# MichelangeloConserva/Colosseum

Hardware: AMD Instinct MI355X
Metric: env steps/sec (whole node) + value-iteration sweeps/sec, DeepSea size=30 x65536 (higher is better)
Workload: dtype i32 state/visit indices, f64 rewards+CDF

## Files before the change

### colosseum_amd/_lib.py

```python
import ctypes as C
import os

import numpy as np

HERE = os.path.dirname(os.path.abspath(__file__))
LIB_PATH = os.path.join(HERE, "libcmdp.so")

OK, ERR_INVALID, ERR_HIP, ERR_NEEDS_RESET, ERR_UNSUPPORTED, ERR_MAX_ITER, ERR_NO_DEVICE, ERR_MAX_VALUE, ERR_OVERFLOW = (
    0, -1, -2, -3, -4, -5, -6, -7, -8)
RNG_MT_COMPAT, RNG_PHILOX = 0, 1
POLICY_RANDOM, POLICY_HOST_ACTIONS, POLICY_GREEDY_Q = 0, 1, 2
POLICY_RANDOM_REFERENCE = 3
SCHEME_AUTO, SCHEME_JACOBI, SCHEME_GAUSS_SEIDEL = 0, 1, 2
LAYOUT_CSR, LAYOUT_DENSE = 0, 1
FLAG_REWARD_MEANS = 1
FLAG_BETA_GAMMAS = 4
FLAG_REWARD_CACHE = 2
OPT_ROLLOUT_KERNEL = 1
OPT_DP_KERNEL = 2
OPT_LDS_GROUPS_PER_CU = 3
OPT_DIAMETER_WORKSPACE_MB = 4
OPT_CHAIN_EXACT_ORDER = 5
OPT_MIXING_PATH = 6
OPT_DIAMETER_RELABEL_MIN_STATES = 7
# ... 5 lines not shown
STAT_UCRL2_WAIT_MS = 16
STAT_PSRL_ROUNDS, STAT_PSRL_SOLVES, STAT_PSRL_SAMPLE_KERNEL_MS, STAT_PSRL_VI_KERNEL_MS, STAT_PSRL_REFERENCE_MS = 17, 18, 19, 20, 21
STAT_DIAMETER_KERNEL = 22
STAT_UCRL2_POLICY_KERNEL_MS = 23
STAT_PSRL_POLICY_KERNEL_MS = 24
STAT_UCRL2_POLICY_SOLVED, STAT_UCRL2_POLICY_REUSED = 25, 26
STAT_ACTIONS_KERNEL_MS = 27
STAT_PSRL_UNCONVERGED, STAT_PSRL_SWEEPS = 28, 29
PSRLC_OPT_SIZE_THRESHOLD, PSRLC_OPT_MAX_SWEEPS, PSRLC_OPT_POLICY_SOLVER = 1, 2, 3
PSRL_SAMPLER_REFERENCE, PSRL_SAMPLER_PHILOX = 0, 1
PSRL_KEY_HI = 0x5053524C
BOUND_CHERNOFF, BOUND_BERNSTEIN = 0, 1
ACTOR_GREEDY, ACTOR_EPSILON_GREEDY, ACTOR_BOLTZMANN = 0, 1, 2
UCRL2_OPT_MAX_SWEEPS = 1
UCRL2_OPT_POLICY_SIZE_THRESHOLD = 2
UCRL2_OPT_POLICY_REUSE = 3
NOISE_NONE, NOISE_GAUSSIAN, NOISE_GAUSSIAN_CORRELATED, NOISE_STUDENT_T, NOISE_STUDENT_T_CORRELATED = 0, 1, 2, 3, 4
CALIB_LDS_READ, CALIB_LDS_CHAIN, CALIB_LDS_CHAIN_SHARED = 0, 1, 2
DP_AUTO, DP_WORKGROUP, DP_REGISTER = 0, 1, 2
DP_REGISTER_DISTINCT = 5
DP_REGISTER_WAVEFRONT = 7
ROLLOUT_AUTO, ROLLOUT_GLOBAL, ROLLOUT_LDS, ROLLOUT_LDS_STOCHASTIC = 0, 1, 2, 3
ROLLOUT_LDS_TEMPLATE = 4
ROLLOUT_LDS_TEMPLATE_STREAM = 5
ROLLOUT_EPISODE_PARALLEL = 6
K1S_PLAN_FIELDS = ("ok", "G", "nw", "gw", "team", "U", "n_pat", "n_codes", "reward_mode", "rc_packed", "n_shapes", "shape_bytes",
                   "ch", "form")
K1S_REWARD_SOURCES = ("packed", "state_table", "row")
K1S_FORMS = {0: "generic", **{t * 4 + i: f"team{t}_{src}" for t in (16, 8, 1) for i, src in enumerate(K1S_REWARD_SOURCES)}}
DET_PLAN_FIELDS = {
    "k1lp": ("ok", "pipe", "packed", "code_shift", "succ_bits", "n_codes", "ch", "G", "per_cu", "capacity", "slot_bytes", "lds_bytes",
             "form"),
    "k1t": ("ok", "automatic", "ch", "G", "capacity", "slot_bytes", "tmpl_bytes", "lds_bytes"),
    "k1u": ("ok", "automatic", "pack10", "ch", "G", "capacity", "lds_bytes", "hist_lds_bytes", "form"),
}
K1LP_FORMS = {0: "k1l_unpacked", 1: "k1l_packed", 2: "k1p"}
K1U_FORMS = {0: "pack10", 1: "wide"}
K1E_PAIR_PLAN_FIELDS = ("ok", "H", "SP2", "n_even", "lds_bytes", "last_form")
K1E_FORMS = {0: None, 1: "single", 2: "pair"}
DET_PLAN_KNOBS = ("pipe", "k1l_G", "k1t_G", "k1u_G", "k1t_ch")

EXPORTS = [
    "cmdp_version", "cmdp_build_id", "cmdp_last_error", "cmdp_device_count", "cmdp_set_device", "cmdp_create", "cmdp_destroy",
    "cmdp_stream", "cmdp_reset", "cmdp_step", "cmdp_rollout", "cmdp_rollout_async", "cmdp_synchronize", "cmdp_stat", "cmdp_calibrate", "cmdp_set_option", "cmdp_lds_plan",
    "cmdp_visits", "cmdp_reset_visits", "cmdp_set_visits", "cmdp_state", "cmdp_last_start", "cmdp_vi_discounted", "cmdp_pe_discounted",
    "cmdp_vi_episodic", "cmdp_pe_episodic", "cmdp_diameter", "cmdp_diameter_episodic", "cmdp_value_norm", "cmdp_gth", "cmdp_qlearning_create", "cmdp_qlearning_destroy", "cmdp_qlearning_run",
    "cmdp_qlearning_tables", "cmdp_qlearning_evaluate", "cmdp_greedy_policy_episodic", "cmdp_qlearning_continuous_create",
    "cmdp_qlearning_policy", "cmdp_qlearning_average_reward", "cmdp_qlearning_run_logged", "cmdp_tracker_replay", "cmdp_average_reward", "cmdp_diameter_range", "cmdp_diameter_sparse_f64", "cmdp_mixing_time", "cmdp_set_observation_table", "cmdp_observe", "cmdp_observe_noise",
    "cmdp_set_reward_streams", "cmdp_legacy_beta", "cmdp_extended_vi",
    "cmdp_ucrl2_create", "cmdp_ucrl2_destroy", "cmdp_ucrl2_run", "cmdp_ucrl2_layout", "cmdp_ucrl2_model", "cmdp_ucrl2_last_solve",
    "cmdp_ucrl2_set_option", "cmdp_ucrl2_policy", "cmdp_ucrl2_average_reward", "cmdp_model_vi_scheme", "cmdp_vi_discounted_model",
    "cmdp_psrl_create", "cmdp_psrl_destroy", "cmdp_psrl_run", "cmdp_psrl_layout", "cmdp_psrl_model", "cmdp_psrl_last_sample",
    "cmdp_psrl_reference_sample", "cmdp_vi_episodic_dense", "cmdp_psrl_episode_end_update", "cmdp_k1e_round_interior",
    "cmdp_k1e_code_counts", "cmdp_k1e_scan_words", "cmdp_k1s_plan", "cmdp_k1s_plan_desc", "cmdp_det_plan", "cmdp_det_plan_desc", "cmdp_chain_plan_desc", "cmdp_chain_choice",
    "cmdp_k1e_pair_plan", "cmdp_k1e_pair_plan_desc",
    "cmdp_psrl_map_rows", "cmdp_vi_episodic_map", "cmdp_psrl_policy", "cmdp_psrl_evaluate",
    "cmdp_ucrl2_run_logged", "cmdp_psrl_run_logged",
    "cmdp_set_action_streams", "cmdp_action_stream_state", "cmdp_set_action_stream_state", "cmdp_mt_randint", "cmdp_mt_action_bits",
    "cmdp_psrlc_create", "cmdp_psrlc_destroy", "cmdp_psrlc_run", "cmdp_psrlc_episode_end_update", "cmdp_psrlc_layout",
    "cmdp_psrlc_model", "cmdp_psrlc_last_sample", "cmdp_psrlc_set_option", "cmdp_psrlc_policy", "cmdp_psrlc_average_reward",
    "cmdp_vi_discounted_dense", "cmdp_vi_discounted_map",
]


class CmdpDesc(C.Structure):
    _fields_ = [
        ("n_instances", C.c_int32), ("n_actions", C.c_int32), ("horizon", C.c_int32), ("rng_mode", C.c_int32),
        ("layout", C.c_int32), ("flags", C.c_int32),
        ("reward_min", C.c_double), ("reward_max", C.c_double),
        ("state_off", C.c_void_p),
        ("sp_ptr", C.c_void_p), ("sp_next", C.c_void_p), ("sp_cum", C.c_void_p), ("sp_reward", C.c_void_p),
        ("sp_rkind", C.c_void_p), ("sp_rp0", C.c_void_p), ("sp_rp1", C.c_void_p), ("sp_seed", C.c_void_p), ("start_off", C.c_void_p), ("start_state", C.c_void_p),
        ("start_cum", C.c_void_p), ("start_seed", C.c_void_p), ("philox_key", C.c_void_p),
        ("csr_ptr", C.c_void_p), ("csr_col", C.c_void_p), ("csr_val", C.c_void_p), ("R", C.c_void_p),
    ]


class CmdpLoopDesc(C.Structure):
    _fields_ = [
        ("n_steps", C.c_int64), ("log_every", C.c_int64),
        ("n_check", C.c_int32), ("horizon", C.c_int32), ("kmax", C.c_int32), ("reserved", C.c_int32),
        ("max_time", C.c_double),
        ("base_val", C.c_void_p), ("base_kind", C.c_void_p), ("opt0", C.c_void_p), ("worst0", C.c_void_p),
        ("start_pos", C.c_void_p), ("start_prob", C.c_void_p),
    ]


LOG_COLUMNS = [
    "cumulative_expected_reward", "cumulative_regret", "cumulative_reward", "normalized_cumulative_expected_reward",
    "normalized_cumulative_regret", "normalized_cumulative_reward", "optimal_cumulative_expected_reward",
    "optimal_normalized_cumulative_expected_reward", "random_cumulative_expected_reward", "random_cumulative_regret",
    "random_normalized_cumulative_expected_reward", "random_normalized_cumulative_regret", "steps_per_second",
    "worst_cumulative_expected_reward", "worst_cumulative_regret", "worst_normalized_cumulative_expected_reward",
    "worst_normalized_cumulative_regret",
]


class CmdpError(RuntimeError):
    def __init__(self, code, message):
        super().__init__(f"libcmdp error {code}: {message}")
        self.code = code


class DynamicProgrammingMaxIterationExceeded(Exception):
    """Same name as the reference's exception (colosseum/dynamic_programming/utils.py:8-9)."""


# ... 88 lines not shown
        L.cmdp_diameter_sparse_f64.argtypes = [vp, C.c_double, i64, vp, vp]
        L.cmdp_mixing_time.argtypes = [vp, vp, vp, C.c_double, i64, vp, vp]
        L.cmdp_set_observation_table.argtypes = [vp, vp, i32, i32]
        L.cmdp_observe.argtypes = [vp, C.c_double, vp]
        L.cmdp_observe_noise.argtypes = [vp, i32, C.c_double, C.c_double, vp, vp]
        L.cmdp_greedy_policy_episodic.argtypes = [vp, i32, i32, vp, vp]
        L.cmdp_qlearning_tables.argtypes = [vp, vp, vp]
        L.cmdp_set_reward_streams.argtypes = [vp, vp, vp, vp, vp]
        L.cmdp_legacy_beta.argtypes = [vp, vp, vp, vp, f64, f64, i64, vp]
        L.cmdp_set_action_streams.argtypes = [vp, vp]
        L.cmdp_action_stream_state.argtypes = [vp, vp, vp]
        L.cmdp_set_action_stream_state.argtypes = [vp, vp, vp]
        L.cmdp_mt_randint.argtypes = [vp, vp, i32, i64, vp]
        L.cmdp_mt_action_bits.argtypes = [vp, vp, i64, i64, vp]
        L.cmdp_ucrl2_create.argtypes = [C.POINTER(vp), vp, vp, i64, f64, f64, i32, i32, i32]
        L.cmdp_ucrl2_destroy.argtypes = [vp]
        L.cmdp_ucrl2_run.argtypes = [vp, i64, i32, vp, vp, vp, vp, vp, vp]
        L.cmdp_ucrl2_layout.argtypes = [vp, vp, vp, vp]
        L.cmdp_ucrl2_model.argtypes = [vp, vp, vp, vp, vp, vp, vp, vp, vp, vp]
        L.cmdp_ucrl2_last_solve.argtypes = [vp, vp, vp, vp, vp, vp, vp, vp, vp, vp]
        L.cmdp_ucrl2_set_option.argtypes = [vp, i32, i64]
        L.cmdp_ucrl2_policy.argtypes = [vp, vp, vp, vp, vp, vp]
        L.cmdp_ucrl2_average_reward.argtypes = [vp, vp, vp, vp]
        L.cmdp_model_vi_scheme.argtypes = [i32, i32, i64, i64, f64]
        L.cmdp_vi_discounted_model.argtypes = [i32, vp, vp, vp, vp, vp, vp, vp, f32, f64, i32, i64, f64, i64, vp, vp, vp, vp, vp]
        L.cmdp_psrl_create.argtypes = [C.POINTER(vp), vp, vp, i64, vp, vp, i32, i32]
        L.cmdp_psrl_destroy.argtypes = [vp]
        L.cmdp_psrl_run.argtypes = [vp, i64, i32, vp, vp, vp, vp, vp, vp]
        L.cmdp_psrl_episode_end_update.argtypes = [vp]
        L.cmdp_psrl_layout.argtypes = [vp, vp, vp, vp]
        L.cmdp_psrl_model.argtypes = [vp, vp, vp, vp, vp]
        L.cmdp_psrl_last_sample.argtypes = [vp, vp, vp, vp]
        L.cmdp_psrl_reference_sample.argtypes = [vp, vp, vp, vp, vp, vp, vp, vp, i32, i32, vp, vp, vp, vp, f32, vp, vp, vp]
        L.cmdp_vi_episodic_dense.argtypes = [i32, vp, vp, i32, vp, vp, vp, vp]
        L.cmdp_psrl_map_rows.argtypes = [i32, i32, vp, vp, vp, f32, vp, vp, vp]
        L.cmdp_vi_episodic_map.argtypes = [i32, vp, vp, i32, vp, vp, vp, vp, vp, vp, vp, vp, vp]
        L.cmdp_psrl_policy.argtypes = [vp, vp, vp, vp]
        L.cmdp_psrl_evaluate.argtypes = [vp, vp, vp]
        L.cmdp_psrlc_create.argtypes = [C.POINTER(vp), vp, vp, i64, vp, vp, i32, i32]
        L.cmdp_psrlc_destroy.argtypes = [vp]
        L.cmdp_psrlc_run.argtypes = [vp, i64, i32, vp, vp, vp, vp, vp, vp]
        L.cmdp_psrlc_episode_end_update.argtypes = [vp]
        L.cmdp_psrlc_layout.argtypes = [vp, vp, vp, vp]
        L.cmdp_psrlc_model.argtypes = [vp, vp, vp, vp, vp, vp, vp]
        L.cmdp_psrlc_last_sample.argtypes = [vp, vp, vp, vp, vp, vp, vp]
        L.cmdp_psrlc_set_option.argtypes = [vp, i32, i64]
        L.cmdp_psrlc_policy.argtypes = [vp, vp, vp, vp, vp, vp]
        L.cmdp_psrlc_average_reward.argtypes = [vp, vp, vp, vp]
        L.cmdp_vi_discounted_dense.argtypes = [i32, vp, vp, vp, vp, f32, f64, i32, i64, f64, i64, vp, vp, vp, vp, vp]
        L.cmdp_vi_discounted_map.argtypes = [i32, vp, vp, vp, vp, vp, vp, vp, f32, f64, i32, i64, f64, i64, vp, vp, vp, vp, vp, vp, vp]
        L.cmdp_k1e_round_interior.argtypes = [i32, i32, i64, i32]
        L.cmdp_k1e_code_counts.argtypes = [C.c_uint32, C.c_uint32, i32]
        L.cmdp_k1e_scan_words.argtypes = [vp, i64, i32, i32, i64, i32, i32, vp, f64, vp, vp]
        L.cmdp_k1s_plan.argtypes = [vp, vp]
        L.cmdp_k1s_plan_desc.argtypes = [C.POINTER(CmdpDesc), i32, i32, vp]
        L.cmdp_det_plan.argtypes = [vp, vp]
        L.cmdp_det_plan_desc.argtypes = [C.POINTER(CmdpDesc), i32, vp, vp]
        L.cmdp_k1e_pair_plan.argtypes = [vp, vp]
        L.cmdp_k1e_pair_plan_desc.argtypes = [C.POINTER(CmdpDesc), i32, i32, vp, vp, vp, vp, vp]
        L.cmdp_chain_plan_desc.argtypes = [C.POINTER(CmdpDesc), vp, vp, vp, vp, i64, vp, vp, vp, vp, vp]
        L.cmdp_chain_choice.argtypes = [i32, i32, i32, i32, i32, vp]
        L.cmdp_k1e_code_counts.restype = C.c_uint32
        _lib = L
    return _lib


def check(rc):
    if rc == OK:
        return
    msg = load().cmdp_last_error().decode()
    if rc == ERR_MAX_ITER:
        raise DynamicProgrammingMaxIterationExceeded(msg)
    if rc == ERR_NEEDS_RESET:
        raise AssertionError(msg)
    raise CmdpError(rc, msg)


def ptr(a):
    return None if a is None else a.ctypes.data_as(C.c_void_p)


def carr(a, dtype):
    return None if a is None else np.ascontiguousarray(a, dtype)


_hip = None


def pinned_empty(n, dtype):
    import weakref

    global _hip
    load()
    if _hip is None:
        _hip = C.CDLL("libamdhip64.so")
        _hip.hipHostMalloc.argtypes = [C.POINTER(C.c_void_p), C.c_size_t, C.c_uint]
        _hip.hipHostFree.argtypes = [C.c_void_p]
    dt = np.dtype(dtype)
    nbytes = max(1, int(n)) * dt.itemsize
    p = C.c_void_p()
    rc = _hip.hipHostMalloc(C.byref(p), nbytes, 0)
    if rc != 0 or not p.value:
        raise MemoryError(f"hipHostMalloc({nbytes}) failed with {rc}")
    buf = (C.c_char * nbytes).from_address(p.value)
    arr = np.frombuffer(buf, dtype=dt, count=int(n))
    weakref.finalize(buf, _hip.hipHostFree, C.c_void_p(p.value))
# ... 2 lines not shown
```

### colosseum_amd/csrc/cmdp.hip

```cpp
#include "../../include/cmdp.h"

#include <hip/hip_runtime.h>
#include <rocblas/rocblas.h>
#include <cstdlib>

#include <algorithm>
#include <chrono>
#include <cstdarg>
#include <limits>
#include <cstdio>
#include <cmath>
#include <cstring>
#include <map>
#include <memory>
#include <mutex>
#include <string>
#include <unordered_map>
#include <vector>

extern char** environ;

#include <new>
#include "cmdp_kernels.h"
#include "cmdp_tracker.h"
// ... 706 lines not shown
  }
  HIP_TRY(h->d_csr_ptr.upload(d->csr_ptr, R + 1, st));
  HIP_TRY(h->d_csr_col.upload(d->csr_col, N, st));
  HIP_TRY(h->d_csr_val.upload(d->csr_val, N, st));
  HIP_TRY(h->d_R.upload(d->R, R, st));
  return CMDP_OK;
}

static int build_dense(cmdp_t* h, const cmdp_desc* d) {
  const int64_t R = h->n_rows;
  for (int64_t k = 0; k < h->n_csr; ++k)
    if (!(d->csr_val[k] >= 3.7252902984619141e-09f) || d->csr_val[k] > 1.0f)
      return fail(CMDP_ERR_INVALID, "dense layout needs probabilities in [2^-28, 1] (entry %lld)", (long long)k);
  const int nv = (h->max_S + 255) / 256;
  const int allowed[] = {1, 2, 3, 4, 6, 8, 12, 16};
  int pick = 0;
  for (int v : allowed) if (v >= nv) { pick = v; break; }
  if (!pick) return fail(CMDP_ERR_UNSUPPORTED, "dense layout supports at most 4096 states per instance");
  h->dense_spad = pick * 256;
  const size_t n = (size_t)R * h->dense_spad;
  size_t free_b = 0, total_b = 0;
  HIP_TRY(hipMemGetInfo(&free_b, &total_b));
  if (n * sizeof(float) > free_b)
    return fail(CMDP_ERR_INVALID, "dense layout needs %zu MiB, %zu MiB free", n * sizeof(float) >> 20, free_b >> 20);
  HIP_TRY(h->d_dense.alloc(n));
  HIP_TRY(h->d_dense.zero(h->stream));
  hipLaunchKernelGGL(k_dense_fill, dim3(grid_for(R, 256)), dim3(256), 0, h->stream, h->d_dense.p, h->dense_spad,
                     h->d_csr_ptr.p, h->d_csr_col.p, h->d_csr_val.p, R);
  HIP_TRY(hipGetLastError());
  return CMDP_OK;
}

extern "C" {

int cmdp_version(void) { return CMDP_ABI_VERSION; }
#ifndef CMDP_BUILD_ID
#define CMDP_BUILD_ID "unstamped"
#endif
static const char k_build_id[] = "CMDP_BUILD_ID=" CMDP_BUILD_ID;
const char* cmdp_build_id(void) { return k_build_id + 14; }

const char* cmdp_last_error(void) { return g_err.c_str(); }

int cmdp_k1e_round_interior(int e_lo, int horizon, int64_t n_steps, int n_instances) {
  return k1e_round_interior(e_lo, horizon, n_steps, n_instances) ? 1 : 0;
}

uint32_t cmdp_k1e_code_counts(uint32_t lo, uint32_t hi, int few) {
  return few ? k1e_code_counts_few(lo, hi) : k1e_code_counts(lo, hi);
}

int cmdp_k1e_scan_words(const uint64_t* words, int64_t n_words, int H, int h0, int64_t n_steps, int nch, int n_codes,
                        const double rv[4], double s0, double* sum, int32_t stats[4]) {
  if (!words || !rv || !sum || !stats) return fail(CMDP_ERR_INVALID, "cmdp_k1e_scan_words: null argument");
  if (H < 1 || h0 < 0 || h0 >= H || n_steps < 1 || n_steps >= ((int64_t)1 << 31) || nch != (H + 31) / 32 || n_codes < 1 || n_codes > 4)
    return fail(CMDP_ERR_INVALID, "cmdp_k1e_scan_words: H %d, h0 %d, n_steps %lld, nch %d, n_codes %d", H, h0, (long long)n_steps, nch, n_codes);
  if ((((int64_t)h0 + n_steps + H - 1) / H) * nch != n_words || n_words >= ((int64_t)1 << 31))
    return fail(CMDP_ERR_INVALID, "cmdp_k1e_scan_words: %lld words do not hold %lld steps from in-episode time %d", (long long)n_words,
                (long long)n_steps, h0);
  double r[4];
  for (int c = 0; c < 4; ++c) r[c] = c < n_codes ? rv[c] : 0.0;
  K1rLane L;
  k1r_init(L, r, n_codes, H, nch, h0, n_steps, s0);
  K1rHostLoader ld{words, L.W};
  K1rStats st;
  k1r_scan(L, ld, st);
  *sum = k1r_sum(L);
  for (int i = 0; i < 4; ++i) stats[i] = st.n[i];
  return CMDP_OK;
}

int cmdp_device_count(void) {
  int n = 0;
  if (hipGetDeviceCount(&n) != hipSuccess) return 0;
  return n;
}

int cmdp_set_device(int device) {
  HIP_TRY(hipSetDevice(device));
  if (const char* e = std::getenv("CMDP_SYNC_MODE")) {
    const unsigned f = !std::strcmp(e, "block") ? hipDeviceScheduleBlockingSync
                     : !std::strcmp(e, "yield") ? hipDeviceScheduleYield
                     : !std::strcmp(e, "spin") ? hipDeviceScheduleSpin : hipDeviceScheduleAuto;
    HIP_TRY(hipSetDeviceFlags(f));
  }
  return CMDP_OK;
}

void* cmdp_stream(cmdp_t* h) { return h ? (void*)h->stream : nullptr; }

int cmdp_destroy(cmdp_t* h) {
  if (h && h->ev_dp0) {
    (void)hipEventDestroy(h->ev_dp0);
    (void)hipEventDestroy(h->ev_dp1);
  }
  if (!h) return CMDP_OK;
  (void)hipSetDevice(h->device);
  if (h->stream) {
    (void)hipStreamSynchronize(h->stream);
    (void)hipStreamDestroy(h->stream);
  }
  for (int i = 0; i < 2; ++i) {
    if (h->aux.walk[i]) (void)hipEventDestroy(h->aux.walk[i]);
    if (h->aux.scan[i]) (void)hipEventDestroy(h->aux.scan[i]);
  }
  if (h->aux.stream) {
    (void)hipStreamSynchronize(h->aux.stream);
    (void)hipStreamDestroy(h->aux.stream);
  }
  for (int i = 0; i < 5; ++i)
    if (h->ev_time[i]) (void)hipEventDestroy(h->ev_time[i]);
  for (int i = 0; i < 2; ++i)
    if (h->ev_row[i]) (void)hipEventDestroy(h->ev_row[i]);
  for (int i = 0; i < 2; ++i)
    if (h->ev_as[i]) (void)hipEventDestroy(h->ev_as[i]);
  for (cmdp_t** back : h->uc_backrefs) *back = nullptr;
  for (double* c : h->rc_chunks) (void)hipFree(c);
  if (h->rc_stage_h) (void)hipHostFree(h->rc_stage_h);
  if (h->rc_dst_h) (void)hipHostFree(h->rc_dst_h);
  if (h->rc_ent_h) (void)hipHostFree(h->rc_ent_h);
  if (h->rc_list_h) (void)hipHostFree(h->rc_list_h);
// ... 4845 lines not shown
```

### colosseum_amd/csrc/cmdp_k1e.h

```cpp
#pragma once

#define K1E_THREADS 1024
#define K1E_NW (K1E_THREADS / 64)
#define K1E_NI 32
#define K1E_EPL 4
#define K1E_EPP (K1E_NW * 2 * K1E_EPL)
#define K1E_SEG 61440
#define K1E_SMASK 0xff80u

struct K1ePlan {
  int32_t S, H;
  int32_t ash;
  int32_t ring_blocks;
  int32_t n_codes;
  int32_t nch;
  int32_t n_pass;
  int32_t gdw;
  int32_t debug;
  int32_t fast;
  const uint32_t* etab;
  const double* rvals;
  uint2* codes;
  int32_t* seg_h0;
  int2* dep;
// ... 408 lines not shown
    }
  }
  __syncthreads();
  const int64_t so0 = t.state_off[g0];
  bool ovf = false;
  auto sat_add = [&](int32_t old, uint32_t add) -> int32_t {
    const int64_t v = (int64_t)old + (int64_t)add;
    if (v > 0x7fffffffLL) { ovf = true; return 0x7fffffff; }
    return (int32_t)v;
  };
  for (int i = wave; i < nb; i += K1E_NW) {
    const int bi = g0 + i;
    const int32_t s_start = t.start_state[t.start_off[bi]];
    const uint32_t n_res = (uint32_t)p.dep_res[bi];
    const int64_t gs0 = so0 + (int64_t)i * S;
    for (int s = lane; s < S; s += 64) {
      const uint32_t c0 = arr0[i * S + s], c1 = arr1[i * S + s];
      const uint32_t add_s = c0 + c1 + (s == s_start ? n_res : 0u);
      if (add_s) t.visits_s[gs0 + s] = sat_add(t.visits_s[gs0 + s], add_s);
      if (c0 | c1) {
        int2* sa = reinterpret_cast<int2*>(t.visits_sa + (gs0 + s) * 2);
        int2 v = *sa;
        v.x = sat_add(v.x, c0);
        v.y = sat_add(v.y, c1);
        *sa = v;
      }
    }
    __builtin_amdgcn_wave_barrier();
    if (lane == 0) p.dep_res[bi] = 0;
  }
  if (ovf) atomicOr(overflow, 1);
}

typedef uint32_t k1r_u32x8 __attribute__((ext_vector_type(8)));
__host__ __device__ __forceinline__ uint32_t k1r_sel8(const k1r_u32x8 a, int i) {
  const bool i0 = (i & 1) != 0, i1 = (i & 2) != 0, i2 = (i & 4) != 0;
  const uint32_t b0 = i0 ? a[1] : a[0], b1 = i0 ? a[3] : a[2], b2 = i0 ? a[5] : a[4], b3 = i0 ? a[7] : a[6];
  const uint32_t c0 = i1 ? b1 : b0, c1 = i1 ? b3 : b2;
  return i2 ? c1 : c0;
}

typedef uint32_t k1r_u32x4 __attribute__((ext_vector_type(4)));
__host__ __device__ __forceinline__ uint32_t k1r_sel8h(const k1r_u32x4 a, int i) {
  const bool i1 = (i & 2) != 0, i2 = (i & 4) != 0;
  const uint32_t b0 = i1 ? a[1] : a[0], b1 = i1 ? a[3] : a[2];
  return ((i2 ? b1 : b0) >> ((i & 1) << 4)) & 0xffffu;
}

#define K1R_THREADS 64
#define K1R_T 8
#define K1R_D 3
#if defined(__HIP_DEVICE_COMPILE__)
#define K1R_ALL(x) (__all(x) != 0)
#else
#define K1R_ALL(x) (x)
#endif

struct K1rNoStats {
  __host__ __device__ __forceinline__ void plain() {}
  __host__ __device__ __forceinline__ void slow() {}
  __host__ __device__ __forceinline__ void word() {}
  __host__ __device__ __forceinline__ void rebase() {}
};
struct K1rStats {
  int32_t n[4] = {0, 0, 0, 0};
  void plain() { ++n[0]; }
  void slow() { ++n[1]; }
  void word() { ++n[2]; }
  void rebase() { ++n[3]; }
};

struct K1rLane {
  double rv[4];
  unsigned long long mv[4];
  int eb[4];
  bool bulk_allowed;
  int n_codes, H, nch;
  int W;
  bool kvalid;
  int kb;
  unsigned long long m;
  uint32_t qlo[4], qhi[4];
  uint32_t tie;
  int ch;
  int e_len;
  int ep_left;
  int tot_left;
};

__host__ __device__ __forceinline__ void k1r_rebase(K1rLane& L) {
  const unsigned long long M52 = (1ull << 52) - 1ull, B52 = 1ull << 52;
  L.kvalid = false;
  const unsigned long long sb = L.m;
  const double S = __builtin_bit_cast(double, sb);
  if (!L.bulk_allowed || !(S >= 2.2250738585072014e-308) || !(S < 1.0e300)) return;
  L.kb = (int)(sb >> 52);
  L.m = (sb & M52) | B52;
  L.tie = 0u;
#pragma unroll
  for (int c = 0; c < 4; ++c) {
    if (c < L.n_codes) {
      unsigned long long qq = 0ull;
      if (L.rv[c] != 0.0) {
        const int d = L.kb - L.eb[c];
        if (L.eb[c] == 0 || d < 0) L.tie |= 1u << c;
        else if (d == 0) qq = L.mv[c];
        else if (d < 55) {
          const unsigned long long half = 1ull << (d - 1), rem = L.mv[c] & ((1ull << d) - 1ull);
          qq = (L.mv[c] >> d) + (rem > half ? 1ull : 0ull);
          if (rem == half) L.tie |= 1u << c;
        }
      }
      L.qlo[c] = (uint32_t)qq;
      L.qhi[c] = (uint32_t)(qq >> 32);
    }
  }
  L.kvalid = true;
}

__host__ __device__ __forceinline__ void k1r_init(K1rLane& L, const double (&rv)[4], int n_codes, int H, int nch, int h0,
                                                  int64_t n_steps, double S0) {
  const unsigned long long M52 = (1ull << 52) - 1ull, B52 = 1ull << 52;
// ... 13 lines not shown
  L.m = __builtin_bit_cast(unsigned long long, S0);
  L.kvalid = false; L.kb = 0; L.tie = 0u;
  L.ch = 0;
  L.e_len = (int)((int64_t)(H - h0) < n_steps ? (int64_t)(H - h0) : n_steps);
  L.ep_left = L.e_len;
  L.tot_left = (int)n_steps;
  k1r_rebase(L);
}

__host__ __device__ __forceinline__ bool k1r_advance(const K1rLane& L, uint32_t n1, uint32_t n2, uint32_t n3, uint32_t steps,
                                                     unsigned long long& m2) {
  const uint32_t n0 = steps - n1 - n2 - n3;
  const uint32_t present = (n0 ? 1u : 0u) | (n1 ? 2u : 0u) | (n2 ? 4u : 0u) | (n3 ? 8u : 0u);
  unsigned long long lo64 = (unsigned long long)n0 * L.qlo[0];
  lo64 += (unsigned long long)n1 * L.qlo[1];
  lo64 += (unsigned long long)n2 * L.qlo[2];
  lo64 += (unsigned long long)n3 * L.qlo[3];
  const uint32_t hi32 = n0 * L.qhi[0] + n1 * L.qhi[1] + n2 * L.qhi[2] + n3 * L.qhi[3];
  m2 = L.m + lo64 + ((unsigned long long)hi32 << 32);
  return L.kvalid && (present & L.tie) == 0u && m2 < (1ull << 53);
}
__host__ __device__ __forceinline__ bool k1r_advance(const K1rLane& L, uint32_t nw, uint32_t steps, unsigned long long& m2) {
  return k1r_advance(L, nw & 0x7ffu, (nw >> 11) & 0x7ffu, nw >> 22, steps, m2);
}
__host__ __device__ __forceinline__ unsigned long long k1r_compose(const K1rLane& L) {
  return ((unsigned long long)L.kb << 52) | (L.m & ((1ull << 52) - 1ull));
}
__host__ __device__ __forceinline__ double k1r_sum(const K1rLane& L) {
  return __builtin_bit_cast(double, L.kvalid ? k1r_compose(L) : L.m);
}

__host__ __device__ __forceinline__ void k1r_tile_counts_few(const k1r_u32x8& clo, const k1r_u32x8& chi, uint32_t& n1, uint32_t& n2) {
  uint32_t n12 = 0u, c2 = 0u;
#pragma unroll
  for (int k = 0; k < K1R_T; ++k) {
    n12 += (uint32_t)__builtin_popcount(clo[k]);
    n12 += (uint32_t)__builtin_popcount(chi[k]);
    c2 += (uint32_t)__builtin_popcount((clo[k] & 0xaaaaaaaau) | ((chi[k] >> 1) & 0x55555555u));
  }
  n1 = n12 - c2; n2 = c2;
}
__host__ __device__ __forceinline__ void k1r_tile_counts(const k1r_u32x8& clo, const k1r_u32x8& chi, uint32_t& n1, uint32_t& n2,
                                                         uint32_t& n3) {
  uint32_t all = 0u, odd = 0u, c3 = 0u;
#pragma unroll
  for (int k = 0; k < K1R_T; ++k) {
    all += (uint32_t)__builtin_popcount(clo[k]);
    all += (uint32_t)__builtin_popcount(chi[k]);
    odd += (uint32_t)__builtin_popcount((clo[k] & 0xaaaaaaaau) | ((chi[k] >> 1) & 0x55555555u));
    const uint32_t l3 = clo[k] & (clo[k] >> 1), h3 = chi[k] & (chi[k] >> 1);
    c3 += (uint32_t)__builtin_popcount((l3 & 0x55555555u) | ((h3 << 1) & 0xaaaaaaaau));
  }
  n3 = c3; n2 = odd - c3; n1 = all - odd - c3;
}

template <class ST>
__host__ __device__ __forceinline__ void k1r_slow(K1rLane& L, const k1r_u32x8& clo, const k1r_u32x8& chi, const k1r_u32x8& P,
                                                  const k1r_u32x4& SP, ST& st) {
  const uint32_t Pt = P[K1R_T - 1], St = SP[K1R_T / 2 - 1] >> 16;
  const double rv0 = L.rv[0], rv1 = L.rv[1], rv2 = L.rv[2], rv3 = L.rv[3];
  unsigned long long m2;
  uint32_t base_n = 0u, base_s = 0u;
  int from = 0;
  for (;;) {
    int lo = from, hi = K1R_T - 1;
#pragma unroll
    for (int it = 0; it < 3; ++it) {
      const int mid = (lo + hi) >> 1;
      const bool ok = k1r_advance(L, k1r_sel8(P, mid) - base_n, k1r_sel8h(SP, mid) - base_s, m2);
      if (lo < hi) { if (ok) lo = mid + 1; else hi = mid; }
    }
    const int k = lo;
    const uint32_t Sk1 = k > 0 ? k1r_sel8h(SP, k - 1) : 0u;
    if (k > from && k1r_advance(L, k1r_sel8(P, k - 1) - base_n, Sk1 - base_s, m2)) L.m = m2;
    const uint32_t Sk = k1r_sel8h(SP, k);
    const uint32_t Lw = Sk - Sk1;
    if (Lw) {
      st.word();
      const uint32_t cx = k1r_sel8(clo, k), cy = k1r_sel8(chi, k);
      double S = __builtin_bit_cast(double, L.kvalid ? k1r_compose(L) : L.m);
#pragma unroll
      for (int half = 0; half < 2; ++half) {
        const uint32_t cw = half ? cy : cx;
        const int Lh = (int)Lw - 16 * half;
        if (Lh > 0) {
          const uint32_t vm = Lh >= 16 ? 0x55555555u : ((1u << (2 * Lh)) - 1u) & 0x55555555u;
          const uint32_t b0 = cw & vm, b1 = (cw >> 1) & vm;
          uint32_t nz = 0u;
          if (rv0 != 0.0) nz |= vm & ~(b0 | b1);
          if (rv1 != 0.0) nz |= b0 & ~b1;
          if (rv2 != 0.0) nz |= b1 & ~b0;
          if (rv3 != 0.0) nz |= b0 & b1;
          while (nz) {
            const uint32_t pos = (uint32_t)__builtin_ctz(nz);
            nz &= nz - 1u;
            const uint32_t cd = cw >> pos;
            const bool c0 = (cd & 1u) != 0u, c1 = (cd & 2u) != 0u;
            const double lo2 = c0 ? rv1 : rv0, hi2 = c0 ? rv3 : rv2;
            S += c1 ? hi2 : lo2;
          }
        }
      }
      L.m = __builtin_bit_cast(unsigned long long, S);
      k1r_rebase(L);
      st.rebase();
    }
    base_n = k1r_sel8(P, k);
    base_s = Sk;
    from = k + 1;
    if (from >= K1R_T) break;
    if (k1r_advance(L, Pt - base_n, St - base_s, m2)) { L.m = m2; break; }
  }
}

template <class ST>
__host__ __device__ __forceinline__ void k1r_tile(K1rLane& L, const k1r_u32x8& clo, const k1r_u32x8& chi, const int w0, ST& st) {
  const int H = L.H;
  const bool few = L.n_codes <= 3;
  unsigned long long m2;
  k1r_u32x8 P;
  k1r_u32x4 SP;
  const bool plain = L.nch == 1 && K1R_ALL(w0 >= 1 && w0 + K1R_T <= L.W - 1);
  if (plain) {
    uint32_t n1, n2, n3;
    bool whole;
    if (few) {
      k1r_tile_counts_few(clo, chi, n1, n2);
      whole = k1r_advance(L, n1, n2, 0u, (uint32_t)(K1R_T * H), m2);
    } else {
      k1r_tile_counts(clo, chi, n1, n2, n3);
      whole = k1r_advance(L, n1, n2, n3, (uint32_t)(K1R_T * H), m2);
    }
    L.tot_left -= K1R_T * H;
    L.e_len = H < L.tot_left ? H : L.tot_left;
    L.ep_left = L.e_len;
    if (whole) { L.m = m2; st.plain(); return; }
  }
  uint32_t rn[K1R_T];
  if (few) {
#pragma unroll
    for (int k = 0; k < K1R_T; ++k) rn[k] = k1e_code_counts_few(clo[k], chi[k]);
  } else {
#pragma unroll
    for (int k = 0; k < K1R_T; ++k) rn[k] = k1e_code_counts(clo[k], chi[k]);
  }
  if (plain) {
    uint32_t acc = 0u;
#pragma unroll
    for (int k = 0; k < K1R_T; ++k) { acc += rn[k]; P[k] = acc; }
#pragma unroll
    for (int k = 0; k < K1R_T; k += 2) SP[k >> 1] = (uint32_t)((k + 1) * H) | ((uint32_t)((k + 2) * H) << 16);
  } else {
    uint32_t acc = 0u, sacc = 0u;
#pragma unroll
    for (int k = 0; k < K1R_T; ++k) {
      const int Lk = (w0 + k < L.W) ? (L.ep_left < 0 ? 0 : (L.ep_left < 32 ? L.ep_left : 32)) : 0;
      acc += Lk > 0 ? rn[k] : 0u;
      sacc += (uint32_t)Lk;
      P[k] = acc;
      if (k & 1) SP[k >> 1] |= sacc << 16; else SP[k >> 1] = sacc;
      L.ep_left -= 32;
      if (++L.ch == L.nch) {
        L.ch = 0;
        L.tot_left -= L.e_len;
        L.e_len = H < L.tot_left ? H : L.tot_left;
        L.ep_left = L.e_len;
      }
    }
    if (k1r_advance(L, P[K1R_T - 1], sacc, m2)) { L.m = m2; return; }
  }
  st.slow();
  k1r_slow(L, clo, chi, P, SP, st);
}

template <class LD, class ST>
__host__ __device__ __forceinline__ void k1r_scan(K1rLane& L, LD& ld, ST& st) {
  k1r_u32x8 loA, hiA, loB, hiB, loC, hiC;
  ld.fetch(loA, hiA, 0);
  ld.fetch(loB, hiB, K1R_T);
  ld.fetch(loC, hiC, 2 * K1R_T);
  const int W = L.W;
  for (int w0 = 0; w0 < W; w0 += K1R_D * K1R_T) {
    k1r_tile(L, loA, hiA, w0, st);
    ld.fetch(loA, hiA, w0 + K1R_D * K1R_T);
    if (w0 + K1R_T < W) {
      k1r_tile(L, loB, hiB, w0 + K1R_T, st);
      ld.fetch(loB, hiB, w0 + (K1R_D + 1) * K1R_T);
    }
    if (w0 + 2 * K1R_T < W) {
      k1r_tile(L, loC, hiC, w0 + 2 * K1R_T, st);
      ld.fetch(loC, hiC, w0 + (K1R_D + 2) * K1R_T);
    }
  }
}

struct K1rHostLoader {
  const uint64_t* words;
  int W;
  void fetch(k1r_u32x8& clo, k1r_u32x8& chi, const int w0) const {
    for (int k = 0; k < K1R_T; ++k) {
      const uint64_t v = w0 + k < W ? words[w0 + k] : 0ull;
      clo[k] = (uint32_t)v; chi[k] = (uint32_t)(v >> 32);
    }
  }
};

typedef uint32_t k1r_u32x2 __attribute__((ext_vector_type(2)));
typedef __attribute__((address_space(1))) unsigned char* k1r_glb_u8;
template <bool OFF32>
struct K1rDeviceLoader {
  k1r_glb_u8 codes;
  uint32_t lane_off;
  int B, W;
  __device__ __forceinline__ const __attribute__((address_space(1))) k1r_u32x2* word(k1r_glb_u8 base, size_t stride, int k) const {
    k1r_glb_u8 wb = base + (size_t)k * stride;
    asm volatile("" : "+s"(wb));
    if constexpr (OFF32) return (const __attribute__((address_space(1))) k1r_u32x2*)(wb + (size_t)lane_off);
    else {
      uint32_t bo = lane_off;
      asm volatile("" : "+v"(bo));
      return (const __attribute__((address_space(1))) k1r_u32x2*)(wb + (size_t)bo * 8);
    }
// ... 46 lines not shown
```

### include/cmdp.h

```cpp
#ifndef CMDP_H
#define CMDP_H

#include <stdint.h>

#ifdef __cplusplus
extern "C" {
#endif

#define CMDP_ABI_VERSION 1

enum {
  CMDP_OK = 0,
  CMDP_ERR_INVALID = -1,
  CMDP_ERR_HIP = -2,
  CMDP_ERR_NEEDS_RESET = -3,
  CMDP_ERR_UNSUPPORTED = -4,
  CMDP_ERR_MAX_ITER = -5,
  CMDP_ERR_NO_DEVICE = -6,
  CMDP_ERR_MAX_VALUE = -7,
  CMDP_ERR_OVERFLOW = -8
};

enum {
  CMDP_RNG_MT_COMPAT = 0,
// ... 14 lines not shown
};

enum {
  CMDP_LAYOUT_CSR = 0,
  CMDP_LAYOUT_DENSE = 1
};

enum {
  CMDP_FLAG_REWARD_MEANS = 1,
  CMDP_FLAG_REWARD_CACHE = 2,
  CMDP_FLAG_BETA_GAMMAS = 4
};

typedef struct cmdp cmdp_t;

typedef struct cmdp_desc {
  int32_t n_instances;
  int32_t n_actions;
  int32_t horizon;
  int32_t rng_mode;
  int32_t layout;
  int32_t flags;
  double reward_min;
  double reward_max;
  const int64_t* state_off;

  const int64_t* sp_ptr;
  const int32_t* sp_next;
  const double*  sp_cum;
  const double*  sp_reward;
  const uint8_t* sp_rkind;
  const double*  sp_rp0;
  const double*  sp_rp1;
  const int32_t* sp_seed;
  const int64_t* start_off;
  const int32_t* start_state;
  const double*  start_cum;
  const int32_t* start_seed;
  const uint64_t* philox_key;

  const int64_t* csr_ptr;
  const int32_t* csr_col;
  const float*   csr_val;
  const float*   R;
} cmdp_desc;

int cmdp_version(void);
const char* cmdp_build_id(void);
const char* cmdp_last_error(void);
int cmdp_k1e_round_interior(int e_lo, int horizon, int64_t n_steps, int n_instances);
uint32_t cmdp_k1e_code_counts(uint32_t lo, uint32_t hi, int few);
int cmdp_k1e_scan_words(const uint64_t* words, int64_t n_words, int H, int h0, int64_t n_steps, int nch, int n_codes,
                        const double rv[4], double s0, double* sum, int32_t stats[4]);
int cmdp_device_count(void);
int cmdp_set_device(int device);

int cmdp_create(cmdp_t** out, const cmdp_desc* desc);
int cmdp_destroy(cmdp_t* h);
void* cmdp_stream(cmdp_t* h);

int cmdp_set_reward_streams(cmdp_t* h, const uint32_t* mt_key, const int32_t* mt_pos, const int32_t* has_gauss,
                            const double* cached_gaussian);
int cmdp_legacy_beta(uint32_t* mt_key, int32_t* mt_pos, int32_t* has_gauss, double* cached_gaussian, double a, double b,
                     int64_t n, double* out);

int cmdp_set_action_streams(cmdp_t* h, const uint32_t* seeds);
int cmdp_action_stream_state(cmdp_t* h, uint32_t* mt_key, int32_t* mt_pos);
int cmdp_set_action_stream_state(cmdp_t* h, const uint32_t* mt_key, const int32_t* mt_pos);
int cmdp_mt_randint(uint32_t* mt_key, int32_t* mt_pos, int n_actions, int64_t n, int8_t* out);
int cmdp_mt_action_bits(uint32_t* mt_key, int32_t* mt_pos, int64_t n, int64_t bit_offset, uint32_t* out);

int cmdp_reset(cmdp_t* h, const uint8_t* mask, int32_t* obs_out);

int cmdp_step(cmdp_t* h, const int32_t* actions, int auto_reset,
              int32_t* obs, double* reward, uint8_t* step_type);

int cmdp_rollout(cmdp_t* h, int policy, const void* policy_arg, int64_t n_steps,
                 int32_t* last_obs, double* reward_sum,
                 int32_t* trace_obs, double* trace_reward, uint8_t* trace_type);
int cmdp_rollout_async(cmdp_t* h, int policy, int64_t n_steps);
int cmdp_synchronize(cmdp_t* h);

enum { CMDP_STAT_DP_KERNEL_MS = 1, CMDP_STAT_DP_KERNEL = 2,
       CMDP_STAT_REWARD_FILLS = 3,
       CMDP_STAT_REWARD_ROUNDS = 4,
       CMDP_STAT_ROLLOUT_KERNEL_MS = 5,
       CMDP_STAT_HIST_KERNEL_MS = 6,
       CMDP_STAT_CHAIN_FAST_INSTANCES = 7 ,
       CMDP_STAT_REWARD_FILL_MS = 8,
       CMDP_STAT_REWARD_ROUND_MS = 9   ,
       CMDP_STAT_DIAMETER_CLUSTER_LAUNCHES = 10,
       CMDP_STAT_DIAMETER_CLUSTER_FALLBACKS = 11  ,
       CMDP_STAT_UCRL2_UNCONVERGED = 12,
       CMDP_STAT_UCRL2_ROUNDS = 13,
       CMDP_STAT_UCRL2_SOLVES = 14,
       CMDP_STAT_UCRL2_ROUND_MS = 15     ,
       CMDP_STAT_UCRL2_WAIT_MS = 16      ,
       CMDP_STAT_PSRL_ROUNDS = 17,
       CMDP_STAT_PSRL_SOLVES = 18,
       CMDP_STAT_PSRL_SAMPLE_KERNEL_MS = 19,
       CMDP_STAT_PSRL_VI_KERNEL_MS = 20,
       CMDP_STAT_PSRL_REFERENCE_MS = 21      ,
       CMDP_STAT_DIAMETER_KERNEL = 22        ,
       CMDP_STAT_UCRL2_POLICY_KERNEL_MS = 23 ,
       CMDP_STAT_PSRL_POLICY_KERNEL_MS = 24  ,
       CMDP_STAT_UCRL2_POLICY_SOLVED = 25,
// ... 191 lines not shown
```

Baseline: 5345 billion.

## Add single-active-reward fast path to k1r tile before slow per-step fallback

```diff
diff --git a/colosseum_amd/_lib.py b/colosseum_amd/_lib.py
--- a/colosseum_amd/_lib.py
+++ b/colosseum_amd/_lib.py
@@ -81,7 +81,7 @@
     "cmdp_ucrl2_set_option", "cmdp_ucrl2_policy", "cmdp_ucrl2_average_reward", "cmdp_model_vi_scheme", "cmdp_vi_discounted_model",
     "cmdp_psrl_create", "cmdp_psrl_destroy", "cmdp_psrl_run", "cmdp_psrl_layout", "cmdp_psrl_model", "cmdp_psrl_last_sample",
     "cmdp_psrl_reference_sample", "cmdp_vi_episodic_dense", "cmdp_psrl_episode_end_update", "cmdp_k1e_round_interior",
-    "cmdp_k1e_code_counts", "cmdp_k1e_scan_words", "cmdp_k1s_plan", "cmdp_k1s_plan_desc", "cmdp_det_plan", "cmdp_det_plan_desc", "cmdp_chain_plan_desc", "cmdp_chain_choice",
+    "cmdp_k1e_code_counts", "cmdp_k1e_scan_words", "cmdp_k1e_scan_words_ex", "cmdp_k1s_plan", "cmdp_k1s_plan_desc", "cmdp_det_plan", "cmdp_det_plan_desc", "cmdp_chain_plan_desc", "cmdp_chain_choice",
     "cmdp_k1e_pair_plan", "cmdp_k1e_pair_plan_desc",
     "cmdp_psrl_map_rows", "cmdp_vi_episodic_map", "cmdp_psrl_policy", "cmdp_psrl_evaluate",
     "cmdp_ucrl2_run_logged", "cmdp_psrl_run_logged",
@@ -276,6 +276,7 @@
         L.cmdp_k1e_round_interior.argtypes = [i32, i32, i64, i32]
         L.cmdp_k1e_code_counts.argtypes = [C.c_uint32, C.c_uint32, i32]
         L.cmdp_k1e_scan_words.argtypes = [vp, i64, i32, i32, i64, i32, i32, vp, f64, vp, vp]
+        L.cmdp_k1e_scan_words_ex.argtypes = [vp, i64, i32, i32, i64, i32, i32, vp, f64, vp, vp]
         L.cmdp_k1s_plan.argtypes = [vp, vp]
         L.cmdp_k1s_plan_desc.argtypes = [C.POINTER(CmdpDesc), i32, i32, vp]
         L.cmdp_det_plan.argtypes = [vp, vp]
diff --git a/colosseum_amd/csrc/cmdp.hip b/colosseum_amd/csrc/cmdp.hip
--- a/colosseum_amd/csrc/cmdp.hip
+++ b/colosseum_amd/csrc/cmdp.hip
@@ -782,6 +782,16 @@
 
 int cmdp_k1e_scan_words(const uint64_t* words, int64_t n_words, int H, int h0, int64_t n_steps, int nch, int n_codes,
                         const double rv[4], double s0, double* sum, int32_t stats[4]) {
+  if (!stats) return fail(CMDP_ERR_INVALID, "cmdp_k1e_scan_words: null argument");
+  int32_t all[8];
+  const int rc = cmdp_k1e_scan_words_ex(words, n_words, H, h0, n_steps, nch, n_codes, rv, s0, sum, all);
+  if (rc != CMDP_OK) return rc;
+  for (int i = 0; i < 4; ++i) stats[i] = all[i];
+  return CMDP_OK;
+}
+
+int cmdp_k1e_scan_words_ex(const uint64_t* words, int64_t n_words, int H, int h0, int64_t n_steps, int nch, int n_codes,
+                           const double rv[4], double s0, double* sum, int32_t stats[8]) {
   if (!words || !rv || !sum || !stats) return fail(CMDP_ERR_INVALID, "cmdp_k1e_scan_words: null argument");
   if (H < 1 || h0 < 0 || h0 >= H || n_steps < 1 || n_steps >= ((int64_t)1 << 31) || nch != (H + 31) / 32 || n_codes < 1 || n_codes > 4)
     return fail(CMDP_ERR_INVALID, "cmdp_k1e_scan_words: H %d, h0 %d, n_steps %lld, nch %d, n_codes %d", H, h0, (long long)n_steps, nch, n_codes);
@@ -796,7 +806,7 @@
   K1rStats st;
   k1r_scan(L, ld, st);
   *sum = k1r_sum(L);
-  for (int i = 0; i < 4; ++i) stats[i] = st.n[i];
+  for (int i = 0; i < 8; ++i) stats[i] = st.n[i];
   return CMDP_OK;
 }
 
diff --git a/colosseum_amd/csrc/cmdp_k1e.h b/colosseum_amd/csrc/cmdp_k1e.h
--- a/colosseum_amd/csrc/cmdp_k1e.h
+++ b/colosseum_amd/csrc/cmdp_k1e.h
@@ -484,8 +484,10 @@
 #define K1R_D 3
 #if defined(__HIP_DEVICE_COMPILE__)
 #define K1R_ALL(x) (__all(x) != 0)
+#define K1R_ANY(x) (__any(x) != 0)
 #else
 #define K1R_ALL(x) (x)
+#define K1R_ANY(x) (x)
 #endif
 
 struct K1rNoStats {
@@ -493,13 +495,19 @@
   __host__ __device__ __forceinline__ void slow() {}
   __host__ __device__ __forceinline__ void word() {}
   __host__ __device__ __forceinline__ void rebase() {}
+  __host__ __device__ __forceinline__ void single() {}
+  __host__ __device__ __forceinline__ void cross() {}
+  __host__ __device__ __forceinline__ void fadd() {}
 };
 struct K1rStats {
-  int32_t n[4] = {0, 0, 0, 0};
+  int32_t n[8] = {0, 0, 0, 0, 0, 0, 0, 0};
   void plain() { ++n[0]; }
   void slow() { ++n[1]; }
   void word() { ++n[2]; }
   void rebase() { ++n[3]; }
+  void single() { ++n[4]; }
+  void cross() { ++n[5]; }
+  void fadd() { ++n[6]; }
 };
 
 struct K1rLane {
@@ -619,6 +627,52 @@
     c3 += (uint32_t)__builtin_popcount((l3 & 0x55555555u) | ((h3 << 1) & 0xaaaaaaaau));
   }
   n3 = c3; n2 = odd - c3; n1 = all - odd - c3;
+}
+
+template <class ST>
+__host__ __device__ __forceinline__ bool k1r_single(K1rLane& L, uint32_t n1, uint32_t n2, uint32_t n3, uint32_t steps, ST& st) {
+  const uint32_t n0 = steps - n1 - n2 - n3;
+  const double rv0 = L.rv[0], rv1 = L.rv[1], rv2 = L.rv[2], rv3 = L.rv[3];
+  const bool a0 = (n0 != 0u) & (rv0 != 0.0), a1 = (n1 != 0u) & (rv1 != 0.0), a2 = (n2 != 0u) & (rv2 != 0.0),
+             a3 = (n3 != 0u) & (rv3 != 0.0);
+  if (!L.bulk_allowed || (int)a0 + (int)a1 + (int)a2 + (int)a3 > 1) return false;
+  st.slow();
+  st.single();
+  uint32_t na = a3 ? n3 : (a2 ? n2 : (a1 ? n1 : (a0 ? n0 : 0u)));
+  const double v = a3 ? rv3 : (a2 ? rv2 : (a1 ? rv1 : rv0));
+  const uint32_t abit = a3 ? 8u : (a2 ? 4u : (a1 ? 2u : 1u));
+  const unsigned long long LIM = 1ull << 53;
+  while (na) {
+    double S;
+    if (!L.kvalid || (L.tie & abit) != 0u) {
+      S = __builtin_bit_cast(double, L.kvalid ? k1r_compose(L) : L.m);
+      for (uint32_t i = 0; i < na; ++i) { S += v; st.fadd(); }
+      na = 0u;
+    } else {
+      const uint32_t ql0 = L.qlo[0], ql1 = L.qlo[1], ql2 = L.qlo[2], ql3 = L.qlo[3];
+      const uint32_t qh0 = L.qhi[0], qh1 = L.qhi[1], qh2 = L.qhi[2], qh3 = L.qhi[3];
+      const uint32_t ql = a3 ? ql3 : (a2 ? ql2 : (a1 ? ql1 : ql0));
+      const uint32_t qh = a3 ? qh3 : (a2 ? qh2 : (a1 ? qh1 : qh0));
+      const unsigned long long q = (unsigned long long)ql | ((unsigned long long)qh << 32);
+      uint32_t j = na;
+      if (q) {
+        const float e = (float)(LIM - 1ull - L.m) / (float)q, en = (float)na;
+        j = (uint32_t)(e < en ? e : en);
+      }
+      unsigned long long t = L.m + (unsigned long long)j * ql + ((unsigned long long)(j * qh) << 32);
+      if (j > 0u && t >= LIM) { --j; t -= q; }
+      else if (j < na && t + q < LIM) { ++j; t += q; }
+      L.m = t;
+      if (j == na) break;
+      S = __builtin_bit_cast(double, k1r_compose(L)) + v;
+      st.cross();
+      na -= j + 1u;
+    }
+    L.m = __builtin_bit_cast(unsigned long long, S);
+    k1r_rebase(L);
+    st.rebase();
+  }
+  return true;
 }
 
 template <class ST>
@@ -688,41 +742,29 @@
   k1r_u32x8 P;
   k1r_u32x4 SP;
   const bool plain = L.nch == 1 && K1R_ALL(w0 >= 1 && w0 + K1R_T <= L.W - 1);
+  uint32_t n1, n2, n3, steps;
+  bool whole;
   if (plain) {
-    uint32_t n1, n2, n3;
-    bool whole;
+    steps = (uint32_t)(K1R_T * H);
     if (few) {
       k1r_tile_counts_few(clo, chi, n1, n2);
-      whole = k1r_advance(L, n1, n2, 0u, (uint32_t)(K1R_T * H), m2);
+      n3 = 0u;
+      whole = k1r_advance(L, n1, n2, 0u, steps, m2);
     } else {
       k1r_tile_counts(clo, chi, n1, n2, n3);
-      whole = k1r_advance(L, n1, n2, n3, (uint32_t)(K1R_T * H), m2);
+      whole = k1r_advance(L, n1, n2, n3, steps, m2);
     }
     L.tot_left -= K1R_T * H;
     L.e_len = H < L.tot_left ? H : L.tot_left;
     L.ep_left = L.e_len;
-    if (whole) { L.m = m2; st.plain(); return; }
-  }
-  uint32_t rn[K1R_T];
-  if (few) {
-#pragma unroll
-    for (int k = 0; k < K1R_T; ++k) rn[k] = k1e_code_counts_few(clo[k], chi[k]);
-  } else {
-#pragma unroll
-    for (int k = 0; k < K1R_T; ++k) rn[k] = k1e_code_counts(clo[k], chi[k]);
-  }
-  if (plain) {
-    uint32_t acc = 0u;
-#pragma unroll
-    for (int k = 0; k < K1R_T; ++k) { acc += rn[k]; P[k] = acc; }
-#pragma unroll
-    for (int k = 0; k < K1R_T; k += 2) SP[k >> 1] = (uint32_t)((k + 1) * H) | ((uint32_t)((k + 2) * H) << 16);
+    if (whole) st.plain();
   } else {
     uint32_t acc = 0u, sacc = 0u;
 #pragma unroll
     for (int k = 0; k < K1R_T; ++k) {
       const int Lk = (w0 + k < L.W) ? (L.ep_left < 0 ? 0 : (L.ep_left < 32 ? L.ep_left : 32)) : 0;
-      acc += Lk > 0 ? rn[k] : 0u;
+      const uint32_t rn = few ? k1e_code_counts_few(clo[k], chi[k]) : k1e_code_counts(clo[k], chi[k]);
+      acc += Lk > 0 ? rn : 0u;
       sacc += (uint32_t)Lk;
       P[k] = acc;
       if (k & 1) SP[k >> 1] |= sacc << 16; else SP[k >> 1] = sacc;
@@ -734,7 +776,23 @@
         L.ep_left = L.e_len;
       }
     }
-    if (k1r_advance(L, P[K1R_T - 1], sacc, m2)) { L.m = m2; return; }
+    n1 = acc & 0x7ffu; n2 = (acc >> 11) & 0x7ffu; n3 = acc >> 22;
+    steps = sacc;
+    whole = k1r_advance(L, n1, n2, n3, steps, m2);
+  }
+  if (whole) { L.m = m2; return; }
+  const bool done = k1r_single(L, n1, n2, n3, steps, st);
+  if (!K1R_ANY(!done)) return;
+  if (done) return;
+  if (plain) {
+    uint32_t acc = 0u;
+#pragma unroll
+    for (int k = 0; k < K1R_T; ++k) {
+      acc += few ? k1e_code_counts_few(clo[k], chi[k]) : k1e_code_counts(clo[k], chi[k]);
+      P[k] = acc;
+    }
+#pragma unroll
+    for (int k = 0; k < K1R_T; k += 2) SP[k >> 1] = (uint32_t)((k + 1) * H) | ((uint32_t)((k + 2) * H) << 16);
   }
   st.slow();
   k1r_slow(L, clo, chi, P, SP, st);
diff --git a/include/cmdp.h b/include/cmdp.h
--- a/include/cmdp.h
+++ b/include/cmdp.h
@@ -90,6 +90,8 @@
 uint32_t cmdp_k1e_code_counts(uint32_t lo, uint32_t hi, int few);
 int cmdp_k1e_scan_words(const uint64_t* words, int64_t n_words, int H, int h0, int64_t n_steps, int nch, int n_codes,
                         const double rv[4], double s0, double* sum, int32_t stats[4]);
+int cmdp_k1e_scan_words_ex(const uint64_t* words, int64_t n_words, int H, int h0, int64_t n_steps, int nch, int n_codes,
+                           const double rv[4], double s0, double* sum, int32_t stats[8]);
 int cmdp_device_count(void);
 int cmdp_set_device(int device);
 
```

New measurement: 5527 billion, median of 6. 1.03x the previous value.
